# auliaadila/LPCNet

Hardware: AMD Instinct MI355X
Metric: real-time 16 kHz streams/GPU; samples/s at batch=1 and batch=1024 (higher is better)
Workload: dtype int8; 1 GPU; BASELINE configs[3]: int8 path, 1024 streams/GPU x 160-sample frames; streams_per_gpu=1024, global_streams=1024, frame_samples=160, parallelism=stream shards x1, no collective

## Files before the change

### lpcnet_amd/csrc/mf_common.h

```cpp
#ifndef LPCNET_MF_COMMON_H
#define LPCNET_MF_COMMON_H

#include <hip/hip_runtime.h>

#include "device_math.h"
#include "lpcnet_engine.h"

namespace lpcnet_mi355x {

typedef int v4i __attribute__((ext_vector_type(4)));

template <int N>
__device__ __forceinline__ void mf_opaque(uint32_t (&o)[N])
{
#pragma unroll
  for (int k = 0; k < N; k++) asm volatile("" : "+v"(o[k]));
}

template <int NO>
__device__ __forceinline__ uint32_t mf_x(const unsigned char *lds, const uint32_t (&o)[NO], int t)
{
  return *(const uint32_t *)(lds + ((o[t >> 1] >> (16 * (t & 1))) & 0xFFFF));
}

__device__ __forceinline__ v4i mfma4(uint32_t x, uint32_t w, v4i acc)
{
  return __builtin_amdgcn_mfma_i32_4x4x4i8((int)x, (int)w, acc, 0, 0, 0);
}

#ifdef MF_SCHED
#define MF_FENCE() __builtin_amdgcn_sched_barrier(0)
#else
#define MF_FENCE() do { } while (0)
#endif

template <int NC>
__device__ __forceinline__ void mf_zr(const unsigned char *lds, const uint32_t (&wz)[MF_ZMAX],
                                      const uint32_t (&wr)[MF_ZMAX], const uint32_t (&oz)[MF_ZMAX / 2],
                                      const uint32_t (&orr)[MF_ZMAX / 2], int ng, v4i (&az)[NC], v4i (&ar)[NC])
{
  uint32_t xz[4], xr[4];
#pragma unroll
  for (int k = 0; k < 4; k++) {
    xz[k] = mf_x(lds, oz, k);
    xr[k] = mf_x(lds, orr, k);
  }
#pragma unroll
  for (int g = 0; g < MF_ZMAX / 4; g++) {
    if (g < ng) {
      uint32_t nz[4], nr[4];
      if (g + 1 < MF_ZMAX / 4 && g + 1 < ng) {
#pragma unroll
        for (int k = 0; k < 4; k++) {
          nz[k] = mf_x(lds, oz, 4 * (g + 1) + k);
          nr[k] = mf_x(lds, orr, 4 * (g + 1) + k);
        }
      }
      MF_FENCE();
#pragma unroll
      for (int k = 0; k < 4; k++) {
        az[k % NC] = mfma4(xz[k], wz[4 * g + k], az[k % NC]);
        ar[k % NC] = mfma4(xr[k], wr[4 * g + k], ar[k % NC]);
      }
      MF_FENCE();
#pragma unroll
      for (int k = 0; k < 4; k++) {
        xz[k] = nz[k];
        xr[k] = nr[k];
      }
    }
  }
}

template <int NS, int NC>
__device__ __forceinline__ void mf_run(const unsigned char *lds, const uint32_t (&w)[NS], const uint32_t (&o)[NS / 2],
                                       int ng, v4i (&a)[NC])
{
  uint32_t x[4];
#pragma unroll
  for (int k = 0; k < 4; k++) x[k] = mf_x(lds, o, k);
#pragma unroll
  for (int g = 0; g < NS / 4; g++) {
    if (g < ng) {
      uint32_t n[4];
      if (g + 1 < NS / 4 && g + 1 < ng) {
#pragma unroll
        for (int k = 0; k < 4; k++) n[k] = mf_x(lds, o, 4 * (g + 1) + k);
      }
      MF_FENCE();
#pragma unroll
      for (int k = 0; k < 4; k++) a[k % NC] = mfma4(x[k], w[4 * g + k], a[k % NC]);
      MF_FENCE();
#pragma unroll
      for (int k = 0; k < 4; k++) x[k] = n[k];
    }
  }
}

template <int NO, int NF>
__device__ __forceinline__ void mf_zr_ct(const unsigned char *lds, const uint32_t (&wz)[MF_ZMAX],
                                         const uint32_t (&wr)[MF_ZMAX], const uint32_t (&oz)[MF_ZMAX / 2],
                                         const uint32_t (&orr)[MF_ZMAX / 2], uint32_t (&xz)[4], uint32_t (&xr)[4],
                                         v4i &az, v4i &ar, v4i &fz, v4i &fr)
{
  static_assert(NO + NF <= MF_ZMAX / 4, "z/r groups");
#pragma unroll
  for (int g = 0; g < NO + NF; g++) {
    uint32_t nz[4], nr[4];
    if (g + 1 < NO + NF) {
#pragma unroll
      for (int k = 0; k < 4; k++) {
        nz[k] = mf_x(lds, oz, 4 * (g + 1) + k);
        nr[k] = mf_x(lds, orr, 4 * (g + 1) + k);
      }
    }
    MF_FENCE();
#pragma unroll
    for (int k = 0; k < 4; k++) {
      if (g < NO) {
        az = mfma4(xz[k], wz[4 * g + k], az);
        ar = mfma4(xr[k], wr[4 * g + k], ar);
      } else {
        fz = mfma4(xz[k], wz[4 * g + k], fz);
        fr = mfma4(xr[k], wr[4 * g + k], fr);
      }
    }
    MF_FENCE();
    if (g + 1 < NO + NF) {
#pragma unroll
      for (int k = 0; k < 4; k++) {
        xz[k] = nz[k];
        xr[k] = nr[k];
      }
    }
  }
}

template <int NO, int NF>
__device__ __forceinline__ void mf_h_ct(const unsigned char *lds, const uint32_t (&w)[MF_HMAX],
                                        const uint32_t (&o)[MF_HMAX / 2], uint32_t (&x)[4], v4i (&a)[2], v4i (&f)[2])
{
  static_assert(NO + NF <= MF_HMAX / 4, "h groups");
#pragma unroll
  for (int g = 0; g < NO + NF; g++) {
    uint32_t n[4];
    if (g + 1 < NO + NF) {
#pragma unroll
      for (int k = 0; k < 4; k++) n[k] = mf_x(lds, o, 4 * (g + 1) + k);
    }
    MF_FENCE();
#pragma unroll
    for (int k = 0; k < 4; k++) {
      if (g < NO)
        a[k & 1] = mfma4(x[k], w[4 * g + k], a[k & 1]);
      else
        f[k & 1] = mfma4(x[k], w[4 * g + k], f[k & 1]);
    }
    MF_FENCE();
    if (g + 1 < NO + NF) {
#pragma unroll
      for (int k = 0; k < 4; k++) x[k] = n[k];
    }
  }
}

#define PIDX(gate, q, row) (((gate) * (NA + 1) + (row)) * (S / 2) + (q))
template <int S, bool PACK>
__device__ __forceinline__ void part_add(int *pg, int gate, int row, const int (&v)[S])
{
  if constexpr (S % 2 == 0 && PACK) {
    unsigned long long *p = (unsigned long long *)pg;
#pragma unroll
    for (int q = 0; q < S / 2; q++)
      atomicAdd(&p[PIDX(gate, q, row)],
                ((unsigned long long)(uint32_t)v[2 * q + 1] << 32) + (unsigned long long)(long long)v[2 * q]);
  } else {
#pragma unroll
    for (int s = 0; s < S; s++) atomicAdd(&pg[(gate * (NA + 1) + row) * S + s], v[s]);
  }
}

template <int S, bool PACK>
__device__ __forceinline__ void part_read(const int *pg, int gate, int row, int (&v)[S])
{
  if constexpr (S % 2 == 0 && PACK) {
    const unsigned long long *p = (const unsigned long long *)pg;
#pragma unroll
    for (int q = 0; q < S / 2; q++) {
      const unsigned long long t = p[PIDX(gate, q, row)];
      const int lo = (int)(uint32_t)t;
      v[2 * q] = lo;
      v[2 * q + 1] = (int)((long long)(t - (unsigned long long)(long long)lo) >> 32);
    }
  } else if constexpr (S == 4) {
    const int4 t = *(const int4 *)&pg[(gate * (NA + 1) + row) * 4];
    v[0] = t.x; v[1] = t.y; v[2] = t.z; v[3] = t.w;
  } else if constexpr (S == 2) {
    const int2 t = *(const int2 *)&pg[(gate * (NA + 1) + row) * 2];
    v[0] = t.x; v[1] = t.y;
  } else {
#pragma unroll
    for (int s = 0; s < S; s++) v[s] = pg[(gate * (NA + 1) + row) * S + s];
  }
}

template <int S, bool PACK>
__device__ __forceinline__ void part_clear(int *pg, int gate, int row)
{
  if constexpr (S % 2 == 0 && PACK) {
    unsigned long long *p = (unsigned long long *)pg;
#pragma unroll
    for (int q = 0; q < S / 2; q++) p[PIDX(gate, q, row)] = 0;
  } else if constexpr (S == 4) {
    *(int4 *)&pg[(gate * (NA + 1) + row) * 4] = make_int4(0, 0, 0, 0);
  } else if constexpr (S == 2) {
    *(int2 *)&pg[(gate * (NA + 1) + row) * 2] = make_int2(0, 0);
  } else {
#pragma unroll
    for (int s = 0; s < S; s++) pg[(gate * (NA + 1) + row) * S + s] = 0;
  }
}

__device__ __forceinline__ void mf_zr_split(const unsigned char *lds, const uint32_t (&wz)[MF_ZMAX],
                                            const uint32_t (&wr)[MF_ZMAX], const uint32_t (&oz)[MF_ZMAX / 2],
                                            const uint32_t (&orr)[MF_ZMAX / 2], int no, int nf, uint32_t (&xz)[4],
                                            uint32_t (&xr)[4], v4i &az, v4i &ar, v4i &fz, v4i &fr)
{
  switch (no * 8 + nf) {
#define MF_ZC(O, F)                                                   \
  case O * 8 + F:                                                     \
    mf_zr_ct<O, F>(lds, wz, wr, oz, orr, xz, xr, az, ar, fz, fr);     \
    break;
    MF_ZC(0, 1) MF_ZC(0, 2) MF_ZC(0, 3) MF_ZC(0, 4)
    MF_ZC(1, 0) MF_ZC(1, 1) MF_ZC(1, 2) MF_ZC(1, 3)
    MF_ZC(2, 0) MF_ZC(2, 1) MF_ZC(2, 2)
    MF_ZC(3, 0) MF_ZC(3, 1)
    MF_ZC(4, 0)
#undef MF_ZC
    default: break;
  }
}

__device__ __forceinline__ void mf_h_split(const unsigned char *lds, const uint32_t (&w)[MF_HMAX],
                                           const uint32_t (&o)[MF_HMAX / 2], int no, int nf, uint32_t (&x)[4],
                                           v4i (&a)[2], v4i (&f)[2])
{
  switch (no * 16 + nf) {
#define MF_HC(O, F)                                \
  case O * 16 + F:                                 \
    mf_h_ct<O, F>(lds, w, o, x, a, f);             \
    break;
    MF_HC(0, 1) MF_HC(0, 2) MF_HC(0, 3) MF_HC(0, 4) MF_HC(0, 5) MF_HC(0, 6) MF_HC(0, 7) MF_HC(0, 8)
    MF_HC(1, 0) MF_HC(1, 1) MF_HC(1, 2) MF_HC(1, 3) MF_HC(1, 4) MF_HC(1, 5) MF_HC(1, 6) MF_HC(1, 7)
    MF_HC(2, 0) MF_HC(2, 1) MF_HC(2, 2) MF_HC(2, 3) MF_HC(2, 4) MF_HC(2, 5) MF_HC(2, 6)
    MF_HC(3, 0) MF_HC(3, 1) MF_HC(3, 2) MF_HC(3, 3) MF_HC(3, 4) MF_HC(3, 5)
    MF_HC(4, 0) MF_HC(4, 1) MF_HC(4, 2) MF_HC(4, 3) MF_HC(4, 4)
    MF_HC(5, 0) MF_HC(5, 1) MF_HC(5, 2) MF_HC(5, 3)
    MF_HC(6, 0) MF_HC(6, 1) MF_HC(6, 2)
    MF_HC(7, 0) MF_HC(7, 1)
    MF_HC(8, 0)
#undef MF_HC
    default: break;
  }
}

template <int S, bool FAST, bool HW, int TB = RCP_TABLE_BITS, typename Stamp>
__device__ __forceinline__ void ga_elementwise(float (&st)[S], const float (&e)[S][9], const float *cnd, int tid,
                                               const float (&faz)[S], const float (&far)[S], const float (&tz)[S],
                                               const float (&tr)[S], const float (&hpre)[S], const uint32_t *rcp,
                                               unsigned char *xa_i, bool stamping, Stamp &stamp)
{
  (void)stamping;
  (void)stamp;
  float zrv[2 * S], hv[S], inh[S];
  for (int s = 0; s < S; s++) {
    const float inz = ((cnd[tid * S + s] + e[s][0]) + e[s][3]) + e[s][6];
    const float inr = ((cnd[(NA + tid) * S + s] + e[s][1]) + e[s][4]) + e[s][7];
    inh[s] = ((cnd[(2 * NA + tid) * S + s] + e[s][2]) + e[s][5]) + e[s][8];
    if (FAST) {
      zrv[s] = (faz[s] + __builtin_rintf((tz[s] + inz) * kScale)) * kScale1;
      zrv[S + s] = (far[s] + __builtin_rintf((tr[s] + inr) * kScale)) * kScale1;
    } else {
      zrv[s] = (float)((int)faz[s] + cvt_rne((tz[s] + inz) * kScale)) * kScale1;
      zrv[S + s] = (float)((int)far[s] + cvt_rne((tr[s] + inr) * kScale)) * kScale1;
    }
    hv[s] = hpre[s];
  }
#ifdef MF_FINE
  if (stamping) { float g = 0.f; for (int k = 0; k < 2 * S; k++) g += zrv[k]; asm volatile("" ::"v"(g)); stamp(11); }
#endif
  sigmoid_x86_fin_n<2 * S, HW, TB>(zrv, rcp);
#ifdef MF_FINE
  if (stamping) { float g = 0.f; for (int k = 0; k < 2 * S; k++) g += zrv[k]; asm volatile("" ::"v"(g)); stamp(12); }
#endif
  for (int s = 0; s < S; s++) hv[s] = hv[s] * zrv[S + s] + inh[s];
  if (FAST)
    tanh_x86_fin_n<S, HW, TB>(hv, rcp);
  else
    tanh_x86_n<S, HW, TB>(hv, rcp);
  for (int s = 0; s < S; s++) st[s] = zrv[s] * st[s] + (1.f - zrv[s]) * hv[s];
#ifdef MF_FINE
  if (stamping) { float g = 0.f; for (int k = 0; k < S; k++) g += st[k]; asm volatile("" ::"v"(g)); stamp(13); }
#endif
  for (int s = 0; s < S; s++) xa_i[s * MF_XSTR] = (unsigned char)quant_s8_state(st[s]);
}

__device__ __forceinline__ v4i mfma16(const v4i &w, const v4i &x, v4i acc)
{
  return __builtin_amdgcn_mfma_i32_16x16x64_i8(w, x, acc, 0, 0, 0);
}


}

#endif
```

### lpcnet_amd/csrc/mf_kernel.hip

```cpp
#include <hip/hip_runtime.h>

#include "device_math.h"
#include "lpcnet_engine.h"
#include "l2_warm.h"
#include "mf_common.h"
#include "sampler.h"

namespace lpcnet_mi355x {

template <int S>
struct MfLds {
  static constexpr int x = S * MF_XSTR;
  static constexpr int xb = S * NB;
  static constexpr int sb = S * NB * 4;
  static constexpr int ix = S * 16;
  static constexpr int pcm = ((S * FRAME * 2 + 15) / 16) * 16;
  static constexpr int cnd = GA_ROWS * S * 4;
  static constexpr int gbs = S * GB_ROWS * 4;
  static constexpr int gbr = GB_ROWS * 4;
  static constexpr int okw = 8 * 4;
  static constexpr int gbw = 3 * 64 * 16;
  static constexpr int total = x + xb + sb + ix + pcm + cnd + gbs + gbr + okw + gbw;
  static constexpr int part = 3 * (NA + 1) * S * 4;
};

int mf_lds_bytes(int S, int split)
{
  const int base = S == 4 ? MfLds<4>::total : (S == 2 ? MfLds<2>::total : MfLds<1>::total);
  const int part = S == 4 ? MfLds<4>::part : (S == 2 ? MfLds<2>::part : MfLds<1>::part);
  return IMG_VAR + base + (split ? part : 0);
}

template <int S, int DIAG, bool SPLIT, bool HWR>
__global__ __launch_bounds__(MF_THREADS) void mf_kernel(SampleArgs A)
{
  constexpr bool TRACE = DIAG == 1;
  extern __shared__ uint4 lds4[];
  unsigned char *lds = (unsigned char *)lds4;
  using L = MfLds<S>;
  unsigned char *xa = lds;
  unsigned char *xb = xa + L::x;
  float *sbuf = (float *)(xb + L::xb);
  int *ix = (int *)((unsigned char *)sbuf + L::sb);
  short *pcmbuf = (short *)((unsigned char *)ix + L::ix);
  float *cnd = (float *)((unsigned char *)pcmbuf + L::pcm);
  int *gbs = (int *)((unsigned char *)cnd + L::cnd);
  int *gbr = gbs + S * GB_ROWS;
  int *okw = gbr + GB_ROWS;
  v4i *gbw = (v4i *)(okw + 8);
  int *part = (int *)(gbw + 3 * 64);
  __shared__ uint4 img_s[IMG_VAR / 16];
  unsigned char *img = (unsigned char *)img_s;

  if (l2_warm_role(A.mf_emb, (A.nstreams + S - 1) / S)) return;
  const int tid = threadIdx.x, lane = tid & 63, wv = __builtin_amdgcn_readfirstlane(tid >> 6);
  const int s0 = blockIdx.x * S;
  const uint32_t *rcp = (const uint32_t *)(img + IMG_RCP);
  constexpr bool kHwA = S == 1 && HWR;
  constexpr bool kGbwLds = S == 4;

  bool active[S];
  bool any = false;
  for (int s = 0; s < S; s++) {
    const int sid = s0 + s;
    active[s] = sid < A.nstreams && frame_count_of(A, sid) > A.delay;
    any |= active[s];
  }
  const int nfr = A.nframes > 1 ? A.nframes : 1;
  const int total = nfr * A.N;
  bool bad = false;
  if (nfr > 1) {
    const FrameCond *cl = A.cond + (size_t)(nfr - 1) * A.nstreams;
    for (int s = 0; s < S; s++) {
      const int sid = s0 + s;
      bad |= sid < A.nstreams && (frame_count_of(A, cl, sid) > A.delay) != active[s];
    }
    if (bad && tid == 0 && A.status) A.status[0] = STATUS_ACTIVITY;
  }
  if (!any || bad) {
    for (int e = tid; e < S * total; e += MF_THREADS) {
      const int s = e / total, fn = e % total, f = fn / A.N, n = fn % A.N;
      if (s0 + s < A.nstreams) A.pcm[((size_t)f * A.nstreams + s0 + s) * A.N + n] = 0;
    }
    return;
  }
  for (int o = tid; o < IMG_VAR / 16; o += MF_THREADS) img_s[o] = A.image[o];
  for (int e = tid; e < S * A.preload; e += MF_THREADS) {
    const int s = e / A.preload, n = e % A.preload;
    pcmbuf[s * FRAME + n] = A.pcm[(size_t)min(s0 + s, A.nstreams - 1) * A.N + n];
  }

  constexpr bool stamping = DIAG == 2;
  unsigned long long stp[16] = {};
  unsigned long long t_prev = 0, t_loop0 = 0;
  auto stamp = [&](int k) {
    if (stamping) {
      const unsigned long long t = __builtin_amdgcn_s_memtime();
      stp[k] += t - t_prev;
      t_prev = t;
    }
  };
  auto stamp_start = [&]() {
    if (stamping) t_prev = t_loop0 = __builtin_amdgcn_s_memtime();
  };

  if (wv < SAMPLE_WAVES) {
    const int i = A.mf_unit[tid];
    const float bz = A.ga_par[i], br = A.ga_par[NA + i], bh = A.ga_par[2 * NA + i];
    const float dz = A.ga_par[3 * NA + i], dr = A.ga_par[4 * NA + i], dh = A.ga_par[5 * NA + i];
    const int wsz = A.ga_wsum[i], wsr = A.ga_wsum[NA + i], wsh = A.ga_wsum[2 * NA + i];
    float st[S];
    for (int s = 0; s < S; s++) st[s] = A.st[min(s0 + s, A.nstreams - 1)].gru_a_state[i];
    auto stage = [&](const FrameCond *cf) {
      bool in_range = true;
      for (int s = 0; s < S; s++) {
        const int sid = min(s0 + s, A.nstreams - 1);
        const float *ca = gru_a_cond_of(cf, A, sid);
        const float cz = ca[i], cr = ca[NA + i], ch = ca[2 * NA + i];
        cnd[tid * S + s] = cz;
        cnd[(NA + tid) * S + s] = cr;
        cnd[(2 * NA + tid) * S + s] = ch;
        in_range &= fabsf(st[s]) <= 2.f && fabsf(cz) <= A.mf_zr_bound && fabsf(cr) <= A.mf_zr_bound &&
                    fabsf(ch) <= A.mf_h_bound;
      }
      if (lane == 0) okw[wv] = __ballot(!in_range) == 0ull;
      for (int e = tid; e < S * GB_ROWS; e += SAMPLE_THREADS) {
        const int s = e / GB_ROWS, r = e % GB_ROWS;
        gbs[e] =
            cvt_rne((A.gb_par[r] + gru_b_cond_of(cf, A, min(s0 + s, A.nstreams - 1))[r]) * kScale) + A.gb_wsum[r];
      }
    };
    const FrameCond *cf = A.cond;
    stage(cf);
    short *pcm_out = A.pcm;
    if (tid < GB_ROWS) gbr[tid] = cvt_rne(A.gb_par[GB_ROWS + tid] * kScale) + A.gb_wsum[GB_ROWS + tid];
    uint32_t wz[MF_ZMAX], wr[MF_ZMAX], wh[MF_HMAX], oz[MF_ZMAX / 2], orr[MF_ZMAX / 2], oh[MF_HMAX / 2];
    {
      const uint32_t *mt = A.mf + (size_t)wv * MF_LANE_U32 * 64 + lane;
#pragma unroll
      for (int t = 0; t < MF_ZMAX; t++) {
        wz[t] = mt[t * 64];
        wr[t] = mt[(MF_ZMAX + t) * 64];
      }
#pragma unroll
      for (int t = 0; t < MF_HMAX; t++) wh[t] = mt[(2 * MF_ZMAX + t) * 64];
      uint32_t cw[MF_GA / 4];
#pragma unroll
      for (int k = 0; k < MF_GA / 4; k++) cw[k] = mt[(MF_GA + k) * 64];
      const uint32_t mo = (uint32_t)min(lane & 3, S - 1) * MF_XSTR;
      auto off = [&](int t) -> uint32_t { return ((cw[t >> 2] >> (8 * (t & 3))) & 0xFF) * 4 + mo; };
#pragma unroll
      for (int t = 0; t < MF_ZMAX / 2; t++) {
        oz[t] = off(2 * t) | (off(2 * t + 1) << 16);
        orr[t] = off(MF_ZMAX + 2 * t) | (off(MF_ZMAX + 2 * t + 1) << 16);
      }
#pragma unroll
      for (int t = 0; t < MF_HMAX / 2; t++) oh[t] = off(2 * MF_ZMAX + 2 * t) | (off(2 * MF_ZMAX + 2 * t + 1) << 16);
    }
    const int nzr = A.mf_nzr[wv], nh = A.mf_nh[wv];
    const int nfzr = SPLIT ? A.mf_nfzr[wv] : 0, nfh = SPLIT ? A.mf_nfh[wv] : 0;
    uint32_t frow = 0;
    if constexpr (SPLIT) {
      const uint32_t *fro = (const uint32_t *)A.mf_frow + tid;
      const uint32_t e0 = fro[0], e1 = fro[SAMPLE_THREADS], e2 = fro[2 * SAMPLE_THREADS];
      frow = (e0 & 0x1FF) | (e1 & 0x1FF) << 9 | (e2 & 0x1FF) << 18 | (e0 >> 16 & 1) << 27 | (e1 >> 16 & 1) << 28 |
             (e2 >> 16 & 1) << 29;
    }

    __syncthreads();
    bool fast = true;
    for (int s = 0; s < S; s++) xa[s * MF_XSTR + i] = (unsigned char)quant_s8_state(st[s]);
    if constexpr (SPLIT)
      for (int e = tid; e < 3 * (NA + 1) * S; e += SAMPLE_THREADS) part[e] = 0;
    __syncthreads();
    stamp_start();
#ifdef MF_PRIO45
    if (wv >= 4) __builtin_amdgcn_s_setprio(MF_PRIO45);
#endif

    int az[S], ar[S], ah[S];
    float faz[S], far[S];
    float tz[S], tr[S], hpre[S];
    auto recurrent = [&]() {
      v4i vz[1] = {{wsz, wsz, wsz, wsz}}, vr[1] = {{wsr, wsr, wsr, wsr}}, vh[2] = {{wsh, wsh, wsh, wsh}, {0, 0, 0, 0}};
      mf_opaque(oz);
      mf_opaque(orr);
      mf_opaque(oh);
      if constexpr (SPLIT) {
        v4i fz = {0, 0, 0, 0}, fr = {0, 0, 0, 0}, fh[2] = {{0, 0, 0, 0}, {0, 0, 0, 0}};
        uint32_t xz[4], xr[4], xh[4];
#pragma unroll
        for (int k = 0; k < 4; k++) {
          xz[k] = mf_x(lds, oz, k);
          xr[k] = mf_x(lds, orr, k);
          xh[k] = mf_x(lds, oh, k);
        }
        mf_zr_split(lds, wz, wr, oz, orr, nzr, nfzr, xz, xr, vz[0], vr[0], fz, fr);
        uint32_t fp = frow;
        asm volatile("" : "+v"(fp));
        const int frz = (int)(fp & 0x1FF), frr = (int)((fp >> 9) & 0x1FF), frh = (int)((fp >> 18) & 0x1FF);
        int pz[S], pr[S], ph[S];
        for (int s = 0; s < S; s++) {
          pz[s] = fz[s];
          pr[s] = fr[s];
        }
        auto padd = [&](int g, int fr_, int (&v)[S]) {
          if constexpr (S < 4) {
            const bool h = fr_ != NA;
            int vv[S];
            for (int s = 0; s < S; s++) vv[s] = h ? v[s] : 0;
            part_add<S, false>(part, g, h ? fr_ : i, vv);
          } else if (fr_ != NA) {
            part_add<S, false>(part, g, fr_, v);
          }
        };
        mf_h_split(lds, wh, oh, nh, nfh, xh, vh, fh);
        for (int s = 0; s < S; s++) ph[s] = fh[0][s] + fh[1][s];
        if (nfzr > 0) {
          padd(0, frz, pz);
          padd(1, frr, pr);
        }
        if (nfh > 0) padd(2, frh, ph);
      } else if (TRACE) {
        mf_zr<1>(lds, wz, wr, oz, orr, nzr, vz, vr);
        mf_run<MF_HMAX, 2>(lds, wh, oh, nh, vh);
      } else {
        switch (nzr * 16 + nh) {
#define MF_CASE(Z, H)                                 \
  case Z * 16 + H:                                    \
    mf_zr<1>(lds, wz, wr, oz, orr, Z, vz, vr);        \
    mf_run<MF_HMAX, 2>(lds, wh, oh, H, vh);           \
    break;
#define MF_CASES(Z) MF_CASE(Z, 1) MF_CASE(Z, 2) MF_CASE(Z, 3) MF_CASE(Z, 4) MF_CASE(Z, 5) MF_CASE(Z, 6) MF_CASE(Z, 7) MF_CASE(Z, 8)
          MF_CASES(1)
          MF_CASES(2)
          MF_CASES(3)
          MF_CASES(4)
#undef MF_CASES
#undef MF_CASE
          default:
            mf_zr<1>(lds, wz, wr, oz, orr, nzr, vz, vr);
            mf_run<MF_HMAX, 2>(lds, wh, oh, nh, vh);
            break;
        }
      }
      for (int s = 0; s < S; s++) {
        az[s] = vz[0][s];
        ar[s] = vr[0][s];
        faz[s] = (float)vz[0][s];
        far[s] = (float)vr[0][s];
        ah[s] = vh[0][s] + vh[1][s];
        tz[s] = bz + dz * st[s];
        tr[s] = br + dr * st[s];
        if constexpr (SPLIT)
          ah[s] += cvt_rne((bh + dh * st[s]) * kScale);
        else
          hpre[s] = (float)(ah[s] + cvt_rne((bh + dh * st[s]) * kScale)) * kScale1;
      }
    };
    recurrent();
    for (int f = 0; f < nfr; f++) {
      if (f > 0) {
        __syncthreads();
        for (int e = tid; e < S * A.N; e += SAMPLE_THREADS) {
          const int s = e / A.N, k = e % A.N;
          if (s0 + s < A.nstreams) pcm_out[(size_t)(s0 + s) * A.N + k] = active[s] ? pcmbuf[s * FRAME + k] : (short)0;
        }
        pcm_out += (size_t)A.nstreams * A.N;
      }
      fast = true;
      for (int w = 0; w < SAMPLE_WAVES; w++) fast &= okw[w] != 0;
      for (int n = 0; n < A.N; n++) {
        stamp(4);
        __syncthreads();
        stamp(5);
        {
          float e[S][9];
          if constexpr (S > 1) {
            int4 ixv[S];
            if constexpr (SPLIT)
              for (int s = 0; s < S; s++) ixv[s] = *(const int4 *)(ix + s * 4);
            for (int s = 0; s < S; s++) {
              const int4 v = SPLIT ? ixv[s] : *(const int4 *)(ix + s * 4);
              uint32_t o1 = (uint32_t)tid * 4u + (uint32_t)v.x;
              uint32_t o2 = (uint32_t)tid * 4u + (uint32_t)v.y;
              uint32_t o3 = (uint32_t)tid * 4u + (uint32_t)v.z;
              asm volatile("" : "+v"(o1), "+v"(o2), "+v"(o3));
              const char *b1 = (const char *)A.mf_emb[0], *b2 = (const char *)A.mf_emb[1], *b3 = (const char *)A.mf_emb[2];
#pragma unroll
              for (uint32_t g = 0; g < 3; g++) {
                e[s][g] = *(const float *)(b1 + o1 + g * NA * 4u);
                e[s][3 + g] = *(const float *)(b2 + o2 + g * NA * 4u);
                e[s][6 + g] = *(const float *)(b3 + o3 + g * NA * 4u);
              }
            }
          } else {
            for (int s = 0; s < S; s++) {
              const int4 v = *(const int4 *)(ix + s * 4);
              const float *e1 = A.mf_emb[0] + (__builtin_amdgcn_readfirstlane(v.x) & 0xFF) * GA_ROWS;
              const float *e2 = A.mf_emb[1] + (__builtin_amdgcn_readfirstlane(v.y) & 0xFF) * GA_ROWS;
              const float *e3 = A.mf_emb[2] + (__builtin_amdgcn_readfirstlane(v.z) & 0xFF) * GA_ROWS;
              uint32_t ub = (uint32_t)tid * 4u;
              asm volatile("" : "+v"(ub));
              const char *b1 = (const char *)e1, *b2 = (const char *)e2, *b3 = (const char *)e3;
#pragma unroll
              for (uint32_t g = 0; g < 3; g++) {
                e[s][g] = *(const float *)(b1 + ub + g * NA * 4u);
                e[s][3 + g] = *(const float *)(b2 + ub + g * NA * 4u);
                e[s][6 + g] = *(const float *)(b3 + ub + g * NA * 4u);
              }
            }
          }
          if constexpr (SPLIT) {
            uint32_t fp = frow;
            asm volatile("" : "+v"(fp));
            int zadd[S], radd[S], hadd[S];
            for (int s = 0; s < S; s++) zadd[s] = radd[s] = hadd[s] = 0;
            if (S < 4) fp |= 7u << 27;
            if (fp >> 27 & 1) {
              part_read<S, false>(part, 0, i, zadd);
              part_clear<S, false>(part, 0, i);
            }
            if (fp >> 28 & 1) {
              part_read<S, false>(part, 1, i, radd);
              part_clear<S, false>(part, 1, i);
            }
            if (fp >> 29 & 1) {
              part_read<S, false>(part, 2, i, hadd);
              part_clear<S, false>(part, 2, i);
            }
            for (int s = 0; s < S; s++) {
              az[s] += zadd[s];
              ar[s] += radd[s];
            }
            for (int s = 0; s < S; s++) {
              hpre[s] = (float)(ah[s] + hadd[s]) * kScale1;
              faz[s] = (float)az[s];
              far[s] = (float)ar[s];
            }
          }
          if (stamping) {
            float g = 0.f;
            for (int s = 0; s < S; s++)
#pragma unroll
              for (int k = 0; k < 9; k++) g += e[s][k];
            asm volatile("" ::"v"(g));
            stamp(10);
          }
          if (__builtin_amdgcn_readfirstlane((int)fast))
            ga_elementwise<S, true, kHwA>(st, e, cnd, tid, faz, far, tz, tr, hpre, rcp, xa + i, stamping, stamp);
          else
            ga_elementwise<S, false, kHwA>(st, e, cnd, tid, faz, far, tz, tr, hpre, rcp, xa + i, stamping, stamp);
        }
        stamp(0);
        __syncthreads();
        stamp(1);
        if (n + 1 < A.N || f + 1 < nfr) recurrent();
        stamp(2);
      }
      if (f + 1 < nfr) {
        cf += A.nstreams;
        stage(cf);
      }
    }
    stamp(4);
    __syncthreads();
    stamp(5);
    for (int s = 0; s < S; s++)
      if (active[s]) A.st[s0 + s].gru_a_state[i] = st[s];
  } else {
    const float *logit_tab = (const float *)(img + IMG_LOGIT);
    const int sw = wv - SAMPLE_WAVES;
    const int half = lane >> 5, hl = lane & 31;
    const int my_s = S == 4 ? 2 * sw + half : sw;
    const bool samp = my_s < S;
    const bool samp_w = samp && (S == 4 || half == 0);
    const int ms = samp ? my_s : 0;
    const bool my_active = samp && s0 + ms < A.nstreams && frame_count_of(A, s0 + ms) > A.delay;
    const int gs = lane >> 4, gu = lane & 15, sl = min(gs, S - 1), sx = min(gu >> 2, S - 1);
    const bool gown = gs < S && (S == 4 ? (gs >> 1) : gs) == sw;
    const bool gact = gown && s0 + gs < A.nstreams && frame_count_of(A, s0 + gs) > A.delay;

    float lsr[NLPC], lpr[NLPC];
    float pred = 0.f, deemph = 0.f;
    uint32_t rz = 0, rw = 0, rj = 0, rc = 0;
    int last_exc = 0;
    {
      const StreamState *p = &A.st[min(s0 + ms, A.nstreams - 1)];
#pragma unroll
      for (int j = 0; j < NLPC; j++) {
        lsr[j] = p->last_sig[j];
        lpr[j] = lpc_of(A, min(s0 + ms, A.nstreams - 1))[j];
      }
      deemph = p->deemph_mem;
      last_exc = p->last_exc & 0xFF;
      rz = p->rng[0]; rw = p->rng[1]; rj = p->rng[2]; rc = p->rng[3];
    }
    float sbv = A.st[min(s0 + sl, A.nstreams - 1)].gru_b_state[gu];
    const bool walk_fin = A.fc_fin && __builtin_amdgcn_readfirstlane((int)(__ballot(!(fabsf(sbv) <= 2.f)) == 0ull));
    constexpr int kRegTiles = kGbwLds ? MF_GB_IN : MF_GB_TILES;
    v4i wt[kRegTiles];
#pragma unroll
    for (int t = 0; t < kRegTiles; t++) {
      const uint4 u = A.mf_gb[t * 64 + lane];
      wt[t] = v4i{(int)u.x, (int)u.y, (int)u.z, (int)u.w};
    }
    if (kGbwLds && sw == 0)
      for (int g = 0; g < 3; g++) {
        const uint4 u = A.mf_gb[(MF_GB_IN + g) * 64 + lane];
        gbw[g * 64 + lane] = v4i{(int)u.x, (int)u.y, (int)u.z, (int)u.w};
      }
    auto put_xb = [&]() {
      if (gown) xb[gs * NB + gu] = (unsigned char)quant_s8_state(sbv);
    };
    __syncthreads();
    FcLane F;
    F.init(img, lane);
    put_xb();
    auto ix_word = [](int su, int pu, int exc) {
      return S > 1 ? make_int4(su * (GA_ROWS * 4), pu * (GA_ROWS * 4), exc * (GA_ROWS * 4), 0) : make_int4(su, pu, exc, 0);
    };
    if (samp) {
      float p2 = 0.f;
#pragma unroll
      for (int j = 0; j < NLPC; j++) p2 = p2 - lsr[j] * lpr[j];
      pred = p2;
      if (samp_w && hl == 0) *(int4 *)(ix + ms * 4) = ix_word(lin2ulaw_x86(lsr[0]), lin2ulaw_x86(pred), last_exc);
    }
    __syncthreads();
    stamp_start();
    __builtin_amdgcn_s_setprio(3);

    float t03 = 0.f, t47 = 0.f;
    constexpr bool tracing = TRACE;
    float pend_pcm = 0.f, pend_pred = 0.f;
    int pend_exc = 0, pend_n = -1;
    auto finish = [&]() {
      if (pend_n < 0) return;
#pragma unroll
      for (int j = NLPC - 1; j > 0; j--) lsr[j] = lsr[j - 1];
      lsr[0] = pend_pcm;
        last_exc = pend_exc;
      pred = pend_pred;
      float o = pend_pcm + kPreemph * deemph;
      deemph = o;
      if (o < -32767) o = -32767;
      if (o > 32767) o = 32767;
      if (samp_w && hl == 0 && pend_n >= A.preload) pcmbuf[ms * FRAME + pend_n] = (short)round_half_up(o);
      put_xb();
      pend_n = -1;
    };
    const FrameCond *cf = A.cond;
    for (int f = 0; f < nfr; f++) {
      if (f > 0) __syncthreads();
      for (int n = 0; n < A.N; n++) {
        stamp(4);
        __syncthreads();
        stamp(5);
        v4i acc[3], accr[3];
        float lpd[NLPC];
        if (samp) {
          finish();
          lpd[0] = 0.f;
#pragma unroll
          for (int j = 1; j < NLPC; j++) lpd[j] = lsr[j - 1] * lpr[j];
          stamp(13);
          const uint32_t r0 = kiss99_next(rz, rw, rj, rc);
          const uint32_t r1 = kiss99_next(rz, rw, rj, rc);
          lane_thresholds(F, logit_tab, r0, r1, t03, t47);
          const v4i xr = *(const v4i *)(xb + sx * NB);
#pragma unroll
          for (int g = 0; g < 3; g++) {
            acc[g] = v4i{gbs[sl * GB_ROWS + 16 * g + gu], 0, 0, 0};
            accr[g] = v4i{gbr[16 * g + gu], 0, 0, 0};
          }
#pragma unroll
          for (int g = 0; g < 3; g++) accr[g] = mfma16(xr, kGbwLds ? gbw[g * 64 + lane] : wt[(MF_GB_IN + g) % kRegTiles], accr[g]);
        }
        stamp(0);
        __syncthreads();
        stamp(1);
        if (!samp) continue;
        {
          v4i xk[6];
#pragma unroll
          for (int kt = 0; kt < 6; kt++) xk[kt] = *(const v4i *)(xa + sx * MF_XSTR + 64 * kt + 16 * gs);
#pragma unroll
          for (int kt = 0; kt < 6; kt++)
#pragma unroll
            for (int g = 0; g < 2; g++) acc[g] = mfma16(xk[kt], wt[g * 6 + kt], acc[g]);
#pragma unroll
          for (int kt = 0; kt < 6; kt++) acc[2] = mfma16(xk[kt], wt[12 + kt], acc[2]);
          stamp(10);
          float zrb[2] = {(float)acc[0][0] * kScale1 + (float)accr[0][0] * kScale1,
                          (float)acc[1][0] * kScale1 + (float)accr[1][0] * kScale1};
          sigmoid_x86_fin_n<2, HWR>(zrb, rcp);
          float hh[1] = {(float)acc[2][0] * kScale1 + ((float)accr[2][0] * kScale1) * zrb[1]};
          stamp(14);
          tanh_x86_fin_n<1, HWR>(hh, rcp);
          sbv = zrb[0] * sbv + (1.f - zrb[0]) * hh[0];
          if (gown) sbuf[gs * NB + gu] = sbv;
        }
        stamp(8);
        __builtin_amdgcn_wave_barrier();
        float xv[NB];
        {
          const float4 *b4 = (const float4 *)(sbuf + ms * NB);
#pragma unroll
          for (int j = 0; j < NB / 4; j++) {
            const float4 v = b4[j];
            xv[4 * j] = v.x; xv[4 * j + 1] = v.y; xv[4 * j + 2] = v.z; xv[4 * j + 3] = v.w;
          }
        }
        stamp(9);
#ifdef MF_WALKFINE
        auto wst = [&](int k, float v) {
          if (stamping) {
            asm volatile("s_waitcnt lgkmcnt(0)" ::: "memory");
            const int u = __builtin_amdgcn_readfirstlane(__float_as_int(v));
            asm volatile("" ::"s"(u));
            stamp(k);
          }
        };
        const WalkOut R = walk_fin ? dual_fc_walk_p<TRACE, true, HWR>(F, t03, t47, xv, pred, lpd, lpr, n < A.preload ? pcmbuf + ms * FRAME + n : nullptr,
                                                                 deemph, wst)
                                   : dual_fc_walk_p<TRACE, false, HWR>(F, t03, t47, xv, pred, lpd, lpr, n < A.preload ? pcmbuf + ms * FRAME + n : nullptr,
                                                                  deemph, wst);
#else
        const short *teach = n < A.preload ? pcmbuf + ms * FRAME + n : nullptr;
        const WalkOut R = walk_fin ? dual_fc_walk_p<TRACE, true, HWR>(F, t03, t47, xv, pred, lpd, lpr, teach, deemph)
                                   : dual_fc_walk_p<TRACE, false, HWR>(F, t03, t47, xv, pred, lpd, lpr, teach, deemph);
#endif
        stamp(11);
        if (samp_w && hl == 0 && n + 1 < A.N) *(int4 *)(ix + ms * 4) = ix_word(R.su, R.pu, R.exc);
        if (tracing && samp_w && hl < 8 && my_active) {
          float v = R.lg[0];
#pragma unroll
          for (int b = 1; b < 8; b++) v = hl == b ? R.lg[b] : v;
          A.trace_logits[((size_t)(s0 + ms) * A.N + n) * 8 + hl] = v;
        }
        if (A.trace_exc && samp_w && hl == 0 && my_active) A.trace_exc[(size_t)(s0 + ms) * A.N + n] = R.exc;
        pend_pcm = R.pcm;
        pend_pred = R.pn;
        pend_exc = R.exc;
        pend_n = n;
        stamp(12);
      }
      if (f + 1 < nfr) {
        finish();
        cf += A.nstreams;
        int lf = lane;
        asm volatile("" : "+v"(lf));
        const int msf = S == 4 ? 2 * sw + (lf >> 5) : sw;
        const float *lp = lpc_of(cf, A, min(s0 + msf, A.nstreams - 1));
#pragma unroll
        for (int j = 0; j < NLPC; j++) lpr[j] = lp[j];
        float p2 = 0.f;
#pragma unroll
        for (int j = 0; j < NLPC; j++) p2 = p2 - lsr[j] * lpr[j];
        pred = p2;
        if (samp_w && hl == 0) *(int4 *)(ix + ms * 4) = ix_word(lin2ulaw_x86(lsr[0]), lin2ulaw_x86(pred), last_exc);
      }
    }
    if (samp) finish();
    stamp(4);
    __syncthreads();
    stamp(5);
    if (samp_w && my_active && hl == 0) {
      StreamState *p = &A.st[s0 + ms];
#pragma unroll
      for (int j = 0; j < NLPC; j++) p->last_sig[j] = lsr[j];
      p->deemph_mem = deemph;
      p->last_exc = last_exc;
      p->rng[0] = rz; p->rng[1] = rw; p->rng[2] = rj; p->rng[3] = rc;
    }
    if (gact) A.st[s0 + gs].gru_b_state[gu] = sbv;
  }
  if (stamping && lane == 0) {
    stp[6] = __builtin_amdgcn_s_memtime() - t_loop0;
    stp[7] = (unsigned long long)total;
    for (int k = 0; k < 16; k++) A.stamps[((size_t)blockIdx.x * STAMP_WAVES + wv) * 16 + k] = stp[k];
  }
  short *pcm_last = A.pcm + (size_t)(nfr - 1) * A.nstreams * A.N;
  for (int e = tid; e < S * A.N; e += MF_THREADS) {
    const int s = e / A.N, n = e % A.N;
    if (s0 + s < A.nstreams) pcm_last[(size_t)(s0 + s) * A.N + n] = active[s] ? pcmbuf[s * FRAME + n] : (short)0;
  }
}

template <int S, int DIAG, bool SPLIT, bool HWR = true>
static int launch_mf_t(const SampleArgs &a, int lds_bytes, hipStream_t stream)
{
  if (ensure_dyn_lds((const void *)mf_kernel<S, DIAG, SPLIT, HWR>, 160 * 1024 - IMG_VAR)) return -1;
  const int grid = warm_grid((a.nstreams + S - 1) / S, a.nstreams);
  hipLaunchKernelGGL((mf_kernel<S, DIAG, SPLIT, HWR>), dim3(grid), dim3(MF_THREADS), lds_bytes - IMG_VAR, stream, a);
  return hipGetLastError() == hipSuccess ? 0 : -1;
}

template <int S>
static int launch_mf_s(const SampleArgs &a, int lds_bytes, hipStream_t st)
{
  if (!a.rcp_hw) {
    if (a.stamps) return -1;
    if (a.mf_split)
      return a.trace_logits ? launch_mf_t<S, 1, true, false>(a, lds_bytes, st) : launch_mf_t<S, 0, true, false>(a, lds_bytes, st);
    return a.trace_logits ? launch_mf_t<S, 1, false, false>(a, lds_bytes, st) : launch_mf_t<S, 0, false, false>(a, lds_bytes, st);
  }
  if (a.mf_split)
    return a.trace_logits ? launch_mf_t<S, 1, true>(a, lds_bytes, st)
           : a.stamps     ? launch_mf_t<S, 2, true>(a, lds_bytes, st)
                          : launch_mf_t<S, 0, true>(a, lds_bytes, st);
  return a.trace_logits ? launch_mf_t<S, 1, false>(a, lds_bytes, st)
         : a.stamps     ? launch_mf_t<S, 2, false>(a, lds_bytes, st)
                        : launch_mf_t<S, 0, false>(a, lds_bytes, st);
}

int launch_mf(const SampleArgs &a, int S, int lds_bytes, void *stream)
{
  hipStream_t st = (hipStream_t)stream;
  if (S == 4) return launch_mf_s<4>(a, lds_bytes, st);
  if (S == 2) return launch_mf_s<2>(a, lds_bytes, st);
  return launch_mf_s<1>(a, lds_bytes, st);
}

}
```

Before: 459.1 million samples/s.

## Stage GRU embedding gathers by gate and overlap arrival with gate math

For four streams per block, the embedding gathers are issued in three groups ordered r, z, h. Explicit s_waitcnt vmcnt waits let the r-gate sigmoid start once its loads land while the z and h loads are still in flight. The aim is to hide global-load latency behind elementwise gate math on the per-sample critical path. The cost is reliance on exact vmcnt counting and sched barriers, which is fragile if the compiler inserts or reorders other vector memory ops.

Measured after the change: 470.7 million samples/s, median of 6. +2.5%, better.

```diff
diff --git a/lpcnet_amd/csrc/mf_common.h b/lpcnet_amd/csrc/mf_common.h
--- a/lpcnet_amd/csrc/mf_common.h
+++ b/lpcnet_amd/csrc/mf_common.h
@@ -305,6 +305,62 @@
   for (int s = 0; s < S; s++) xa_i[s * MF_XSTR] = (unsigned char)quant_s8_state(st[s]);
 }
 
+template <int N>
+__device__ __forceinline__ void ga_arrived(float (&v)[4][3])
+{
+  asm volatile("s_waitcnt vmcnt(%12)"
+               : "+v"(v[0][0]), "+v"(v[0][1]), "+v"(v[0][2]), "+v"(v[1][0]), "+v"(v[1][1]), "+v"(v[1][2]),
+                 "+v"(v[2][0]), "+v"(v[2][1]), "+v"(v[2][2]), "+v"(v[3][0]), "+v"(v[3][1]), "+v"(v[3][2])
+               : "n"(N)
+               : "memory");
+}
+
+template <int S, bool FAST, bool HW, int TB = RCP_TABLE_BITS, typename Stamp>
+__device__ __forceinline__ void ga_elementwise_staged(float (&st)[S], float (&e)[3][S][3], const float *cnd, int tid,
+                                                      const float (&faz)[S], const float (&far)[S],
+                                                      const float (&tz)[S], const float (&tr)[S],
+                                                      const float (&hpre)[S], const uint32_t *rcp,
+                                                      unsigned char *xa_i, bool stamping, Stamp &stamp)
+{
+  static_assert(S == 4, "staged form: four streams per lane (ga_arrived)");
+  (void)stamping;
+  (void)stamp;
+  float c[3][S];
+  for (int g = 0; g < 3; g++)
+    for (int s = 0; s < S; s++) c[g][s] = cnd[(g * NA + tid) * S + s];
+  auto pre = [](const float (&ev)[3], float cv, float fa, float t) {
+    const float in = ((cv + ev[0]) + ev[1]) + ev[2];
+    return FAST ? (fa + __builtin_rintf((t + in) * kScale)) * kScale1
+                : (float)((int)fa + cvt_rne((t + in) * kScale)) * kScale1;
+  };
+  auto fine = [&](int k, const float(&v)[S]) {
+#ifdef MF_FINE
+    if (stamping) { float g = 0.f; for (int j = 0; j < S; j++) g += v[j]; asm volatile("" ::"v"(g)); stamp(k); }
+#endif
+  };
+  float rv[S], zv[S], hv[S];
+  ga_arrived<6 * S>(e[0]);
+  if (stamping) stamp(10);
+  for (int s = 0; s < S; s++) rv[s] = pre(e[0][s], c[1][s], far[s], tr[s]);
+  sigmoid_x86_fin_n<S, HW, TB>(rv, rcp);
+  fine(11, rv);
+  __builtin_amdgcn_sched_barrier(0);
+  ga_arrived<3 * S>(e[1]);
+  for (int s = 0; s < S; s++) zv[s] = pre(e[1][s], c[0][s], faz[s], tz[s]);
+  sigmoid_x86_fin_n<S, HW, TB>(zv, rcp);
+  fine(12, zv);
+  __builtin_amdgcn_sched_barrier(0);
+  ga_arrived<0>(e[2]);
+  for (int s = 0; s < S; s++) hv[s] = hpre[s] * rv[s] + (((c[2][s] + e[2][s][0]) + e[2][s][1]) + e[2][s][2]);
+  if (FAST)
+    tanh_x86_fin_n<S, HW, TB>(hv, rcp);
+  else
+    tanh_x86_n<S, HW, TB>(hv, rcp);
+  for (int s = 0; s < S; s++) st[s] = zv[s] * st[s] + (1.f - zv[s]) * hv[s];
+  fine(13, st);
+  for (int s = 0; s < S; s++) xa_i[s * MF_XSTR] = (unsigned char)quant_s8_state(st[s]);
+}
+
 __device__ __forceinline__ v4i mfma16(const v4i &w, const v4i &x, v4i acc)
 {
   return __builtin_amdgcn_mfma_i32_16x16x64_i8(w, x, acc, 0, 0, 0);
diff --git a/lpcnet_amd/csrc/mf_kernel.hip b/lpcnet_amd/csrc/mf_kernel.hip
--- a/lpcnet_amd/csrc/mf_kernel.hip
+++ b/lpcnet_amd/csrc/mf_kernel.hip
@@ -57,6 +57,7 @@
   const int s0 = blockIdx.x * S;
   const uint32_t *rcp = (const uint32_t *)(img + IMG_RCP);
   constexpr bool kHwA = S == 1 && HWR;
+  constexpr bool kStaged = S == 4;
   constexpr bool kGbwLds = S == 4;
 
   bool active[S];
@@ -275,8 +276,30 @@
         __syncthreads();
         stamp(5);
         {
-          float e[S][9];
-          if constexpr (S > 1) {
+          [[maybe_unused]] float e[S][9];
+          [[maybe_unused]] float eg[3][S][3];
+          if constexpr (kStaged) {
+            int4 ixv[S];
+            for (int s = 0; s < S; s++) ixv[s] = *(const int4 *)(ix + s * 4);
+            uint32_t o[S][3];
+            for (int s = 0; s < S; s++) {
+              o[s][0] = (uint32_t)tid * 4u + (uint32_t)ixv[s].x;
+              o[s][1] = (uint32_t)tid * 4u + (uint32_t)ixv[s].y;
+              o[s][2] = (uint32_t)tid * 4u + (uint32_t)ixv[s].z;
+            }
+            const char *b1 = (const char *)A.mf_emb[0], *b2 = (const char *)A.mf_emb[1], *b3 = (const char *)A.mf_emb[2];
+#pragma unroll
+            for (int k = 0; k < 3; k++) {
+              const uint32_t g = k < 2 ? 1 - k : k;
+              for (int s = 0; s < S; s++) asm volatile("" : "+v"(o[s][0]), "+v"(o[s][1]), "+v"(o[s][2]));
+              for (int s = 0; s < S; s++) {
+                eg[k][s][0] = *(const float *)(b1 + o[s][0] + g * NA * 4u);
+                eg[k][s][1] = *(const float *)(b2 + o[s][1] + g * NA * 4u);
+                eg[k][s][2] = *(const float *)(b3 + o[s][2] + g * NA * 4u);
+              }
+              __builtin_amdgcn_sched_barrier(0);
+            }
+          } else if constexpr (S > 1) {
             int4 ixv[S];
             if constexpr (SPLIT)
               for (int s = 0; s < S; s++) ixv[s] = *(const int4 *)(ix + s * 4);
@@ -339,7 +362,7 @@
               far[s] = (float)ar[s];
             }
           }
-          if (stamping) {
+          if (stamping && !kStaged) {
             float g = 0.f;
             for (int s = 0; s < S; s++)
 #pragma unroll
@@ -347,7 +370,22 @@
             asm volatile("" ::"v"(g));
             stamp(10);
           }
-          if (__builtin_amdgcn_readfirstlane((int)fast))
+#ifdef MF_ARRIVAL
+          if constexpr (stamping && kStaged) {
+            __builtin_amdgcn_sched_barrier(0);
+            ga_arrived<6 * S>(eg[0]);
+            stamp(8);
+            ga_arrived<3 * S>(eg[1]);
+            stamp(9);
+            ga_arrived<0>(eg[2]);
+          }
+#endif
+          if constexpr (kStaged) {
+            if (__builtin_amdgcn_readfirstlane((int)fast))
+              ga_elementwise_staged<S, true, kHwA>(st, eg, cnd, tid, faz, far, tz, tr, hpre, rcp, xa + i, stamping, stamp);
+            else
+              ga_elementwise_staged<S, false, kHwA>(st, eg, cnd, tid, faz, far, tz, tr, hpre, rcp, xa + i, stamping, stamp);
+          } else if (__builtin_amdgcn_readfirstlane((int)fast))
             ga_elementwise<S, true, kHwA>(st, e, cnd, tid, faz, far, tz, tr, hpre, rcp, xa + i, stamping, stamp);
           else
             ga_elementwise<S, false, kHwA>(st, e, cnd, tid, faz, far, tz, tr, hpre, rcp, xa + i, stamping, stamp);
```
